# ctpeterson/qex

Hardware: AMD Instinct MI355X
Metric: staggered Dslash GFLOP/s + CG iters/s, 32^4 SU(3) fp64, 1/2/4/8 MI355X (higher is better)
Workload: dtype f64

## Files before the change

qex_amd/csrc/dslash.hip:

```cpp
#include "qexhip_internal.h"
#include "site_index.h"
#include "reduce.h"
#include "fused_sweep.h"
#include <hip/hip_ext.h>
#include <cstring>
#include <algorithm>
#include <chrono>

static double now_us() { return std::chrono::duration<double, std::micro>(std::chrono::steady_clock::now().time_since_epoch()).count(); }

struct DslashArgs {
  Geom g;
  const double2 *W;
  const unsigned long long *S;
  const double2 *in;
  double2 *out;
  const double2 *rin;
  const double2 *xs;
  double ca, cb;
  double sgn;
  double post;
  int parity, c0, c1;
  int d0, d1, nb1;
  const double2 *gh_hi, *gh_lo;
  double *partials;
  const int *done;
  int swz;
  int ntstore;
  FusedSweep fs;
};

#include "dslash_core.h"

template <int NDIR, bool HALO, bool INIT, bool DOT, int RECON, bool FUSED>
__device__ __forceinline__ void dslash_body(const DslashArgs &A) {
  const bool skip = A.done && *A.done;
  if (skip && !FUSED) return;
  if (FUSED && fused_push(A.fs, skip)) return;
  FusedRole R;
  R.bid = blockIdx.x; R.cleanup = false; R.bnd = false; R.parked = false;
  if (FUSED) fused_enter(A.fs, A.nb1, R);
  const bool cleanup = FUSED && R.cleanup;
  for (;;) {
    int lb = R.bid;
    if (FUSED && !fused_next_block(A.fs, R, lb)) break;
    const bool bnd = FUSED && R.bnd;
    if (A.swz && !bnd) {
      int per = A.swz >> 3;
      lb = (lb & 7) * per + (lb >> 3);
    }
    int c = A.c0 + lb * 256 + threadIdx.x;
    int clim = A.c1;
    if (FUSED) c = fused_site(A.fs, R, lb, A.c0, A.c1, A.d0, A.d1, clim);
    else if (lb >= A.nb1) { c = A.d0 + (lb - A.nb1) * 256 + threadIdx.x; clim = A.d1; }
    double dotv = 0;
    const bool active = c < clim && !skip;
    const Geom &g = A.g;
    const SiteXYZT s = site_coord(g, c, A.parity);
    const int tu = FUSED ? __builtin_amdgcn_readfirstlane(s.t) : 0;
    double2 acc[3];
    double2 xsv[3];
    constexpr int NLOAD = (RECON == 1 || RECON == 3) ? 6 : (RECON == 2 ? 7 : 9);
    constexpr int LROW = RECON == 3 ? LR_ROW : NLOAD * 64;
    const double2 *w = A.W + (size_t)(c >> 6) * (NDIR * LROW) + (c & 63);
    const unsigned long long *sm = RECON == 1 ? A.S + (size_t)(c >> 6) * NDIR : (RECON == 3 ? A.S + (size_t)(c >> 6) * NDIR * 2 : nullptr);
    const double2 *in_f1 = A.in, *in_b1 = A.in, *in_f3 = A.in, *in_b3 = A.in;
    if (FUSED) {
      in_f1 = tu + 1 >= g.X[3] ? A.gh_hi : A.in;
      in_b1 = tu - 1 < 0 ? A.gh_lo : A.in;
      in_f3 = tu + 3 >= g.X[3] ? A.gh_hi : A.in;
      in_b3 = tu - 3 < 0 ? A.gh_lo : A.in;
    }
    auto pair = [&](const int pr, const bool do_f, const bool do_b) __attribute__((always_inline)) {
      const int mu = pr & 3;
      const int hop = pr >= 4 ? 3 : 1;
      const int pf = nbr_pos<HALO>(g, c, s, mu, hop);
      const int pb = nbr_pos<HALO>(g, c, s, mu, -hop);
      const double2 *wp = w + (size_t)pr * (2 * LROW);
      double2 U[9], W[9], vf[3], vb[3];
      if (do_f) {
#pragma unroll
        for (int k = 0; k < NLOAD; k++) {
          d2v t = __builtin_nontemporal_load((const d2v *)&wp[k * 64]);
          U[k] = make_double2(t.x, t.y);
        }
      }
      if (do_b) {
#pragma unroll
        for (int k = 0; k < NLOAD; k++) {
          d2v t = __builtin_nontemporal_load((const d2v *)&wp[LROW + k * 64]);
          W[k] = make_double2(t.x, t.y);
        }
      }
      if (RECON == 1) {
        const int lane = c & 63;
        if (do_f) recon_row2<1>(U, (sm[2 * pr] >> lane) & 1ull);
        if (do_b) recon_row2<1>(W, (sm[2 * pr + 1] >> lane) & 1ull);
      } else if (RECON == 3) {
        const int lane = c & 63;
        const size_t fr = ((size_t)(c >> 6) * NDIR + 2 * pr) * 576 + lane;
        if (do_f) recon_row2_res(U, wp - lane, sm + 4 * pr, A.S - 2, fr, lane);
        if (do_b) recon_row2_res(W, wp - lane + LROW, sm + 4 * pr + 2, A.S - 2, fr + 576, lane);
      } else if (RECON == 2) {
        if (do_f) recon_row2<2>(U, false);
        if (do_b) recon_row2<2>(W, false);
      }
      const double2 *srcf = (FUSED && mu == 3) ? (hop == 3 ? in_f3 : in_f1) : A.in;
      const double2 *srcb = (FUSED && mu == 3) ? (hop == 3 ? in_b3 : in_b1) : A.in;
      if (do_f) {
#pragma unroll
        for (int k = 0; k < 3; k++) vf[k] = srcf[vec_off(pf, k)];
      }
      if (do_b) {
#pragma unroll
        for (int k = 0; k < 3; k++) vb[k] = srcb[vec_off(pb, k)];
      }
      if (do_f) mv3<false>(acc, U, vf);
      if (do_b) mv3<true>(acc, W, vb);
    };
    auto edge_pairs = [&](const bool crossing) __attribute__((always_inline)) {
      if (!crossing) {
        constexpr int NSP = NDIR / 2 - NDIR / 8;
        constexpr int UNS = NDIR == 8 ? 1 : 2;
#pragma unroll UNS
        for (int q = 0; q < NSP; q++) pair(q + q / 3, true, true);
      }
#pragma unroll 1
      for (int pr = 3; pr < NDIR / 2; pr += 4) {
        const int hop = pr >= 4 ? 3 : 1;
        const bool xf = tu + hop >= g.X[3], xb = tu - hop < 0;
        pair(pr, crossing ? xf : !xf, crossing ? xb : !xb);
      }
    };
    const bool edge = FUSED && bnd;
    if (active) {
      if ((INIT && !cleanup) || DOT) {
#pragma unroll
        for (int k = 0; k < 3; k++) xsv[k] = A.xs[vec_off(c, k)];
      }
      if (FUSED && cleanup) {
#pragma unroll
        for (int k = 0; k < 3; k++) acc[k] = A.out[vec_off(c, k)];
      } else if (INIT) {
#pragma unroll
        for (int k = 0; k < 3; k++) {
          acc[k].x = (A.sgn * A.cb) * xsv[k].x;
          acc[k].y = (A.sgn * A.cb) * xsv[k].y;
        }
        if (A.ca != 0.0) {
#pragma unroll
          for (int k = 0; k < 3; k++) {
            double2 r = A.rin[vec_off(c, k)];
            acc[k].x += (A.sgn * A.ca) * r.x;
            acc[k].y += (A.sgn * A.ca) * r.y;
          }
        }
      } else {
#pragma unroll
        for (int k = 0; k < 3; k++) acc[k] = make_double2(0.0, 0.0);
      }
      constexpr int UNR = (NDIR == 8) ? (RECON == 3 ? (FUSED ? 1 : 2) : (RECON ? 1 : 4)) : 2;
      if (!edge) {
#pragma unroll UNR
        for (int pr = 0; pr < NDIR / 2; pr++) pair(pr, true, true);
      } else if (!cleanup) {
        edge_pairs(false);
      }
    }
    if (edge && !skip) {
      fused_wait_faces(A.fs, R);
      if (active && !R.parked) edge_pairs(true);
    }
    const bool parked = FUSED && R.parked;
    if (active) {
      if (parked) {
#pragma unroll
        for (int k = 0; k < 3; k++) A.out[vec_off(c, k)] = acc[k];
      } else {
#pragma unroll
        for (int k = 0; k < 3; k++) {
          acc[k].x *= (A.sgn * A.post); acc[k].y *= (A.sgn * A.post);
          if (A.ntstore) {
            d2v t; t.x = acc[k].x; t.y = acc[k].y;
            __builtin_nontemporal_store(t, (d2v *)&A.out[vec_off(c, k)]);
          } else {
            A.out[vec_off(c, k)] = acc[k];
          }
        }
        if (DOT) {
#pragma unroll
          for (int k = 0; k < 3; k++) dotv = fma(xsv[k].x, acc[k].x, fma(xsv[k].y, acc[k].y, dotv));
        }
      }
    }
    if (DOT && !skip && !parked) {
      const int pidx = !FUSED ? (RECON == 3 ? lb : (int)blockIdx.x) : fused_partial_slot(A.fs, R, lb);
      double r = block_sum_256(dotv);
      if (threadIdx.x == 0) A.partials[pidx] = r;
    }
    if (!cleanup) break;
  }
  if (FUSED) fused_finish(A.fs, R);
}

template <int NDIR, bool HALO, bool INIT, bool DOT, int RECON>
__global__ void __launch_bounds__(256) k_dslash(DslashArgs A) { dslash_body<NDIR, HALO, INIT, DOT, RECON, false>(A); }
template <int NDIR, bool INIT, bool DOT, int RECON>
__global__ void __launch_bounds__(256) k_dslash_fused(DslashArgs A) { dslash_body<NDIR, true, INIT, DOT, RECON, true>(A); }

template <class K>
static void launch_timed(qexhip_ctx *c, const char *tname, K kernel, dim3 grid, dim3 block, DslashArgs &A, hipStream_t st) {
  hipEvent_t e0 = nullptr, e1 = nullptr;
  if (timer_event_pair(c, tname, &e0, &e1)) hipExtLaunchKernelGGL(kernel, grid, block, 0, st, e0, e1, 0, A);
  else hipLaunchKernelGGL(kernel, grid, block, 0, st, A);
}

template <int NDIR, bool HALO>
static int launch(qexhip_ctx *c, DslashArgs &A, int c0, int c1, bool init, bool dot, int part_off,
                  int d0 = 0, int d1 = 0, const char *tname = "dslash", hipStream_t st = nullptr, int fused_grid = 0) {
  if (!st) st = c->stream;
  const bool fused = fused_grid > 0;
  if (c1 <= c0 && d1 <= d0) return 0;
  if (c1 <= c0) { c0 = d0; c1 = d1; d0 = d1 = 0; }
  A.c0 = c0; A.c1 = c1; A.d0 = d0; A.d1 = d1;
  A.nb1 = (c1 - c0 + 255) / 256;
  const int nb = A.nb1 + (d1 > d0 ? (d1 - d0 + 255) / 256 : 0);
  const int nsw = fused ? A.nb1 : nb;
  A.swz = ((c->recon != 0 || (c->lres && !fused)) && nsw >= 64 && (nsw & 7) == 0) ? nsw : 0;
  A.ntstore = 1;
  double *psave = A.partials;
  A.partials = psave ? psave + part_off : nullptr;
  dim3 grid(fused ? fused_grid : nb), block(256);
#define QX_LAUNCH(R) \
  do { \
    if (HALO && fused) { \
      if (init && dot) launch_timed(c, tname, k_dslash_fused<NDIR, true, true, R>, grid, block, A, st); \
      else if (init) launch_timed(c, tname, k_dslash_fused<NDIR, true, false, R>, grid, block, A, st); \
      else if (dot) launch_timed(c, tname, k_dslash_fused<NDIR, false, true, R>, grid, block, A, st); \
      else launch_timed(c, tname, k_dslash_fused<NDIR, false, false, R>, grid, block, A, st); \
    } else if (init && dot) launch_timed(c, tname, k_dslash<NDIR, HALO, true, true, R>, grid, block, A, st); \
    else if (init) launch_timed(c, tname, k_dslash<NDIR, HALO, true, false, R>, grid, block, A, st); \
    else if (dot) launch_timed(c, tname, k_dslash<NDIR, HALO, false, true, R>, grid, block, A, st); \
    else launch_timed(c, tname, k_dslash<NDIR, HALO, false, false, R>, grid, block, A, st); \
  } while (0)
  if (c->recon == 1) QX_LAUNCH(1);
  else if (c->recon == 2) QX_LAUNCH(2);
  else if constexpr (NDIR == 8) {
    if (c->lres) QX_LAUNCH(3);
    else QX_LAUNCH(0);
  } else QX_LAUNCH(0);
#undef QX_LAUNCH
  A.partials = psave;
  HIPCHK(hipGetLastError());
  return 0;
}

void sweep_plan(const qexhip_ctx *c, int *lo_end_out, int *hi_beg_out, int *overlap_out) {
  const Geom &g = c->g;
  int lo_end = g.depth * g.F; if (lo_end > g.Vh) lo_end = g.Vh;
  int hi_beg = g.Vh - g.depth * g.F; if (hi_beg < lo_end) hi_beg = lo_end;
  const size_t face_bytes = (size_t)g.depth * g.F * 48;
  *lo_end_out = lo_end; *hi_beg_out = hi_beg;
  const int tuned = c->overlap_auto[c->ndir == 16];
  *overlap_out = !g.halo || hi_beg <= lo_end ? 0
                 : (c->opt_overlap >= 0 ? (c->opt_overlap != 0)
                    : (tuned >= 0 ? tuned : ((hi_beg - lo_end) >= 131072 && face_bytes >= ((size_t)1 << 20))));
}

int sweep_form(const qexhip_ctx *c, int overlap) {
  if (!overlap || !peer_faces(c)) return 0;
  if (c->opt_hop_split >= 0) return c->opt_hop_split ? 2 : 0;
  const int m = c->form_auto[c->ndir == 16];
  return m >= 0 ? m : 2;
}

static double exchange_estimate_us(const qexhip_ctx *c) {
  const double meas = c->xchg_us[c->ndir == 16];
  if (meas > 0) return meas;
  const double link = (c->emu_link_gbs > 0 ? c->emu_link_gbs : 45.0) * 1e3;
  return 3.0 + (double)c->g.depth * c->g.F * 48.0 / link;
}
double sweep_push_fraction(const qexhip_ctx *c, int interior_sites, int nrhs) {
  const double bsite = c->ndir * (c->recon == 1 ? 96.0 : (c->recon == 2 ? 112.0 : (c->lres ? 108.0 : 144.0))) + 120.0 * nrhs;
  const double t_int = (double)interior_sites * bsite / 5.5e6;
  return t_int > 0 ? std::min(1.0, std::max(0.65, nrhs * exchange_estimate_us(c) / t_int)) : 1.0;
}

static int sweep_fused_ctl(qexhip_ctx *c, int nbnd, FusedCtl *F, int nrhs) {
  if (c->fz_cap < nbnd) {
    HIPCHK(hipStreamSynchronize(c->stream));
    if (c->fz_buf) HIPCHK(hipFree(c->fz_buf));
    c->fz_buf = nullptr; c->fz_cap = 0;
    const int cap = std::max(2 * nbnd, 4096);
    HIPCHK(hipMalloc((void **)&c->fz_buf, (size_t)(256 + cap) * sizeof(unsigned int)));
    HIPCHK(hipMemsetAsync(c->fz_buf, 0, (size_t)(256 + cap) * sizeof(unsigned int), c->stream));
    c->fz_cap = cap;
  }
  F->dec = c->fz_buf; F->ndef = c->fz_buf + 32; F->cl_done = c->fz_buf + 64; F->late = c->fz_buf + 96;
  F->list = c->fz_buf + 256;
  F->ncl = std::max(std::min(nbnd, 4), std::min(nbnd / 8, 32));
  const double tick_per_us = (double)c->dj.ticks / (c->dj.timeout_s * 1e6);
  if (c->opt_fused_spin_us == -2) F->spin_ticks = -1;
  else {
    const double us = c->opt_fused_spin_us >= 0 ? (double)c->opt_fused_spin_us : std::max(25.0, nrhs * exchange_estimate_us(c));
    F->spin_ticks = (long long)(us * tick_per_us);
  }
  return 0;
}

int fused_sweep_setup(qexhip_ctx *c, int nrhs, DevField *const *f, int parity, int lo_end, int hi_beg, FusedSweep *F,
                      const double2 **gh_hi, const double2 **gh_lo, int *grid, int *nparts) {
  const int nb_int = (hi_beg - lo_end + 255) / 256, nb_lo = (lo_end + 255) / 256, nb_hi = (c->g.Vh - hi_beg + 255) / 256;
  CHK(comm_halo_push_only_multi(c, nrhs, f, parity, gh_hi, gh_lo, &F->push));
  CHK(peer_ghost_args(c, &F->pg));
  CHK(sweep_fused_ctl(c, nb_lo + nb_hi, &F->fz, nrhs));
  F->e0 = hi_beg; F->e1 = c->g.Vh; F->nb2 = nb_int + nb_lo;
  F->nbA = (int)(sweep_push_fraction(c, hi_beg - lo_end, nrhs) * nb_int);
// ... 162 lines not shown
```

qex_amd/csrc/dslash_core.h:

```cpp
#pragma once
#include <hip/hip_runtime.h>
#include "link_residual.h"

typedef double d2v __attribute__((ext_vector_type(2)));

template <bool SUB>
__device__ __forceinline__ void mv3(double2 acc[3], const double2 U[9], const double2 v[3]) {
#pragma unroll
  for (int i = 0; i < 3; i++) {
#pragma unroll
    for (int j = 0; j < 3; j++) {
      if (!SUB) {
        acc[i].x += U[3 * i + j].x * v[j].x;
        acc[i].x -= U[3 * i + j].y * v[j].y;
        acc[i].y += U[3 * i + j].x * v[j].y;
        acc[i].y += U[3 * i + j].y * v[j].x;
      } else {
        acc[i].x -= U[3 * i + j].x * v[j].x;
        acc[i].x += U[3 * i + j].y * v[j].y;
        acc[i].y -= U[3 * i + j].x * v[j].y;
        acc[i].y -= U[3 * i + j].y * v[j].x;
      }
    }
  }
}

template <int FMT>
__device__ __forceinline__ void recon_row2(double2 U[9], bool neg) {
  const double2 ph = U[6];
  double2 r2[3];
#pragma unroll
  for (int k = 0; k < 3; k++) {
    const int a = (k + 1) % 3, b = (k + 2) % 3;
    double rx = U[a].x * U[3 + b].x;
    rx -= U[a].y * U[3 + b].y;
    rx -= U[b].x * U[3 + a].x;
    rx += U[b].y * U[3 + a].y;
    double ry = U[b].x * U[3 + a].y;
    ry += U[b].y * U[3 + a].x;
    ry -= U[a].x * U[3 + b].y;
    ry -= U[a].y * U[3 + b].x;
    if (FMT == 1) r2[k] = make_double2(neg ? -rx : rx, neg ? -ry : ry);
    else r2[k] = make_double2(fma(ph.x, rx, -(ph.y * ry)), fma(ph.x, ry, ph.y * rx));
  }
#pragma unroll
  for (int k = 0; k < 3; k++) U[6 + k] = r2[k];
}

__device__ __forceinline__ void recon_row2_res(double2 U[9], const double2 *row, const unsigned long long *m, const unsigned long long *hdr,
                                               size_t fr, int lane) {
  const uint64_t lo = __builtin_nontemporal_load((const uint64_t *)(row + LR_RES) + lane);
  const uint32_t hi = __builtin_nontemporal_load((const uint32_t *)(row + LR_RES + 32) + lane);
  double2 r2[3];
  lr_decode(U, (m[0] >> lane) & 1ull, lo, hi, r2);
  if ((m[1] >> lane) & 1ull) {
    const double2 *wf = (const double2 *)(uintptr_t)hdr[0] + fr;
#pragma unroll
    for (int k = 0; k < 3; k++) r2[k] = wf[(6 + k) * 64];
  }
#pragma unroll
  for (int k = 0; k < 3; k++) U[6 + k] = r2[k];
}

template <int RECON>
__device__ __forceinline__ void load_link(double2 U[9], const double2 *w, const unsigned long long *sm, int lane) {
  constexpr int NLOAD = RECON == 1 ? 6 : (RECON == 2 ? 7 : 9);
#pragma unroll
  for (int k = 0; k < NLOAD; k++) U[k] = w[k * 64];
  if (RECON == 1) recon_row2<1>(U, (*sm >> lane) & 1ull);
  else if (RECON == 2) recon_row2<2>(U, false);
}
```

qex_amd/csrc/layout.hip:

```cpp
#include <algorithm>
#include <vector>
#include "qexhip_internal.h"
#include "site_index.h"
#include "link_residual.h"
#include <cstring>

int geom_init(Geom &g, const int X[4], int depth, int halo) {
  for (int i = 0; i < 4; i++) {
    if (X[i] < 2 || (X[i] & 1)) { qexhip_set_error("local lattice extents must be even and >= 2 (got %d in dim %d)", X[i], i); return -1; }
    if (X[i] > 1024) { qexhip_set_error("local lattice extents above 1024 are not supported (got %d in dim %d)", X[i], i); return -1; }
    g.X[i] = X[i];
  }
  g.Xh = X[0] / 2;
  g.V = X[0] * X[1] * X[2] * X[3];
  g.Vh = g.V / 2;
  g.F = g.Xh * X[1] * X[2];
  g.ntile = (g.Vh + QEXHIP_TILE - 1) / QEXHIP_TILE;
  g.halo = halo;
  g.depth = halo ? depth : 0;
  if (halo) {
    if (g.F % QEXHIP_TILE) { qexhip_set_error("sharding in t needs X*Y*Z/2 to be a multiple of 64 (got %d)", g.F); return -1; }
    if (X[3] < 3) { qexhip_set_error("sharding in t needs a local t extent >= 3"); return -1; }
    g.gtile = 3 * g.F / QEXHIP_TILE;
  } else {
// ... 37 lines not shown

int field_upload(qexhip_ctx *c, DevField &f, const double *host) {
  size_t bytes = (size_t)c->g.V * 6 * sizeof(double);
  CHK(ensure_stage(c, bytes));
  HIPCHK(hipMemcpyAsync(c->stage, host, bytes, hipMemcpyHostToDevice, c->stream));
  k_vec_to_tiles<<<(c->g.V + 255) / 256, 256, 0, c->stream>>>(c->g, (const double2 *)c->stage, f.d, f.half);
  HIPCHK(hipGetLastError());
  return 0;
}

int field_download(qexhip_ctx *c, const DevField &f, double *host) {
  size_t bytes = (size_t)c->g.V * 6 * sizeof(double);
  CHK(ensure_stage(c, bytes));
  k_vec_from_tiles<<<(c->g.V + 255) / 256, 256, 0, c->stream>>>(c->g, (double2 *)c->stage, f.d, f.half);
  HIPCHK(hipGetLastError());
  HIPCHK(hipMemcpyAsync(host, c->stage, bytes, hipMemcpyDeviceToHost, c->stream));
  HIPCHK(hipStreamSynchronize(c->stream));
  return 0;
}

__global__ void __launch_bounds__(256) k_pack_top_links(Geom g, const double2 *__restrict__ hostfmt, double2 *buf) {
  int n = g.depth * g.F;
  int i = blockIdx.x * 256 + threadIdx.x;
  if (i >= 2 * n) return;
  int p = i / n, j = i - p * n;
  int c = g.Vh - n + j;
  const double2 *U = hostfmt + ((size_t)(p * g.Vh + c) * 4 + 3) * 9;
  for (int k = 0; k < 9; k++) buf[(size_t)i * 9 + k] = U[k];
}

template <bool HALO>
__global__ void __launch_bounds__(256) k_links_to_tiles(Geom g, const double2 *__restrict__ hostfmt,
                                                        const double2 *__restrict__ ghost, double2 *W,
                                                        int ndir, int dbase, int hop) {
  int i = blockIdx.x * 256 + threadIdx.x;
  if (i >= g.V) return;
  int p = i >= g.Vh, c = i - p * g.Vh;
  SiteXYZT s = site_coord(g, c, p);
  double2 *w = W + ((size_t)p * g.ntile + (c >> 6)) * ndir * 576 + (c & 63);
  for (int mu = 0; mu < 4; mu++) {
    const double2 *U = hostfmt + ((size_t)i * 4 + mu) * 9;
    double2 *wf = w + (size_t)(dbase + 2 * mu) * 576;
    for (int k = 0; k < 9; k++) wf[k * 64] = U[k];
    const double2 *B;
    if (HALO && mu == 3 && s.t - hop < 0) {
      int cF = c - s.t * g.F;
      int j = (s.t - hop + g.depth) * g.F + cF;
      B = ghost + ((size_t)(1 - p) * g.depth * g.F + j) * 9;
    } else {
      int cb = nbr_pos<false>(g, c, s, mu, -hop);
      B = hostfmt + ((size_t)((1 - p) * g.Vh + cb) * 4 + mu) * 9;
    }
    double2 *wb = w + (size_t)(dbase + 2 * mu + 1) * 576;
    for (int r = 0; r < 3; r++)
      for (int q = 0; q < 3; q++) {
        double2 v = B[q * 3 + r];
        wb[(r * 3 + q) * 64] = make_double2(v.x, -v.y);
      }
  }
}

int links_upload(qexhip_ctx *c, const double *fat, const double *lng) {
  c->cg_resume.valid = 0;
  const Geom &g = c->g;
  int ndir = lng ? 16 : 8;
  if (lng) for (int i = 0; i < 4; i++) if (g.X[i] < 4) { qexhip_set_error("Naik links need local extents >= 4"); return -1; }
  if (lng && g.halo && g.depth < 3) { qexhip_set_error("internal: ghost depth %d < 3 for Naik links", g.depth); return -3; }
  size_t wbytes = (size_t)2 * g.ntile * ndir * 576 * sizeof(double2);
  if (c->W && c->ndir != ndir) { HIPCHK(hipFree(c->W)); c->W = nullptr; }
  if (!c->W) { HIPCHK(hipMalloc((void **)&c->W, wbytes)); }
  HIPCHK(hipMemsetAsync(c->W, 0, wbytes, c->stream));
  c->ndir = ndir;
  size_t gbytes = (size_t)g.V * 72 * sizeof(double);
  size_t ghost_elems = g.halo ? (size_t)2 * g.depth * g.F * 9 : 0;
  size_t ghost_bytes = ghost_elems * sizeof(double2);
  CHK(ensure_stage(c, gbytes + 2 * ghost_bytes + 256));
  double2 *hostfmt = (double2 *)c->stage;
  double2 *sendbuf = (double2 *)((char *)c->stage + gbytes);
  double2 *ghost = (double2 *)((char *)c->stage + gbytes + ghost_bytes);
  for (int pass = 0; pass < (lng ? 2 : 1); pass++) {
    const double *src = pass ? lng : fat;
    HIPCHK(hipMemcpyAsync(hostfmt, src, gbytes, hipMemcpyHostToDevice, c->stream));
    if (g.halo) {
      int n = 2 * g.depth * g.F;
      k_pack_top_links<<<(n + 255) / 256, 256, 0, c->stream>>>(g, hostfmt, sendbuf);
      HIPCHK(hipGetLastError());
      CHK(comm_exchange_raw(c, sendbuf, ghost, ghost_bytes, c->stream));
      k_links_to_tiles<true><<<(g.V + 255) / 256, 256, 0, c->stream>>>(g, hostfmt, ghost, c->W, ndir, pass * 8, pass ? 3 : 1);
    } else {
      k_links_to_tiles<false><<<(g.V + 255) / 256, 256, 0, c->stream>>>(g, hostfmt, nullptr, c->W, ndir, pass * 8, pass ? 3 : 1);
    }
    HIPCHK(hipGetLastError());
  }
  HIPCHK(hipStreamSynchronize(c->stream));
  CHK(links_compress(c));
  return sweep_autotune(c);
}

template <int FMT>
__global__ void __launch_bounds__(256) k_links_compress(size_t nrows, const double2 *__restrict__ W, double2 *Wc,
                                                        unsigned long long *Ws, unsigned int *maxdev) {
  const size_t j = (size_t)blockIdx.x * 256 + threadIdx.x;
  const size_t row = j >> 6;
  if (row >= nrows) return;
  const int l = j & 63;
  const double2 *w = W + row * 576 + l;
  constexpr int NR = FMT == 1 ? 6 : 7;
  double2 *o = Wc + row * (NR * 64) + l;
  double2 u[9], r[3];
#pragma unroll
  for (int k = 0; k < 9; k++) u[k] = w[k * 64];
#pragma unroll
  for (int k = 0; k < 6; k++) o[k * 64] = u[k];
  double n2 = 0, px = 0, py = 0;
#pragma unroll
  for (int k = 0; k < 3; k++) {
    const int a = (k + 1) % 3, b = (k + 2) % 3;
    r[k].x = (u[a].x * u[3 + b].x - u[a].y * u[3 + b].y) - (u[b].x * u[3 + a].x - u[b].y * u[3 + a].y);
    r[k].y = -((u[a].x * u[3 + b].y + u[a].y * u[3 + b].x) - (u[b].x * u[3 + a].y + u[b].y * u[3 + a].x));
    n2 += r[k].x * r[k].x + r[k].y * r[k].y;
    px += u[6 + k].x * r[k].x + u[6 + k].y * r[k].y;
    py += u[6 + k].y * r[k].x - u[6 + k].x * r[k].y;
  }
  double2 ph;
  if (n2 > 0) ph = make_double2(px / n2, py / n2); else ph = make_double2(1.0, 0.0);
  if (FMT == 1) ph = make_double2(ph.x < 0 ? -1.0 : 1.0, 0.0);
  double dev = 0;
#pragma unroll
  for (int k = 0; k < 3; k++) {
    const double rx = ph.x * r[k].x - ph.y * r[k].y, ry = ph.x * r[k].y + ph.y * r[k].x;
    dev = fmax(dev, fmax(fabs(u[6 + k].x - rx), fabs(u[6 + k].y - ry)));
  }
  if (FMT == 1) {
    const unsigned long long mask = __ballot(ph.x < 0);
    if (l == 0) Ws[row] = mask;
  } else {
    o[6 * 64] = ph;
  }
  unsigned int bits = __float_as_uint((float)dev);
#pragma unroll
  for (int off = 32; off > 0; off >>= 1) {
    const unsigned int o2 = __shfl_xor(bits, off, 64);
    bits = o2 > bits ? o2 : bits;
  }
  if (l == 0 && bits > __hip_atomic_load(maxdev, __ATOMIC_RELAXED, __HIP_MEMORY_SCOPE_AGENT)) atomicMax(maxdev, bits);
}
__global__ void __launch_bounds__(256) k_links_residual(size_t nrows, size_t prows, const double2 *__restrict__ W, double2 *Wc,
                                                        unsigned long long *Wm, unsigned int *nesc) {
  const size_t j = (size_t)blockIdx.x * 256 + threadIdx.x;
  const size_t row = j >> 6;
  if (row >= nrows) return;
  const int l = j & 63;
  const double2 *w = W + row * 576 + l;
  double2 *o = Wc + row * LR_ROW + l;
  double2 u[9];
#pragma unroll
  for (int k = 0; k < 9; k++) u[k] = w[k * 64];
#pragma unroll
  for (int k = 0; k < 6; k++) o[k * 64] = u[k];
  bool neg;
  uint64_t lo;
  uint32_t hi;
  const bool ok = lr_encode(u, &neg, &lo, &hi);
  ((uint64_t *)(Wc + row * LR_ROW + LR_RES))[l] = lo;
  ((uint32_t *)(Wc + row * LR_ROW + LR_RES + 32))[l] = hi;
  const unsigned long long sgn = __ballot(neg), esc = __ballot(!ok);
  if (l == 0) {
    unsigned long long *m = Wm + 2 * (row + row / prows + 1);
    m[0] = sgn;
    m[1] = esc;
    if (esc) atomicAdd(nesc, (unsigned int)__popcll(esc));
  }
}

int link_residual_host(const double2 *u, long n, unsigned char *escaped, double2 *row2) {
  for (long i = 0; i < n; i++) {
    bool neg;
    uint64_t lo;
    uint32_t hi;
    const bool ok = lr_encode(u + 9 * i, &neg, &lo, &hi);
    if (escaped) escaped[i] = !ok;
    if (row2) lr_decode(u + 9 * i, neg, lo, hi, row2 + 3 * i);
  }
  return 0;
}

int links_compress(qexhip_ctx *c) {
  const Geom &g = c->g;
  c->links_gen++;
  c->recon = 0;
  c->lres = 0; c->lres_esc = 0;
  if (!c->opt_recon || !c->W) return 0;
  const size_t nrows = (size_t)2 * g.ntile * c->ndir;
  if (c->Wc_rows < nrows) {
    if (c->Wc) HIPCHK(hipFree(c->Wc));
    if (c->Ws) HIPCHK(hipFree(c->Ws));
    HIPCHK(hipMalloc((void **)&c->Wc, nrows * 448 * sizeof(double2)));
    HIPCHK(hipMalloc((void **)&c->Ws, nrows * sizeof(unsigned long long)));
    c->Wc_rows = nrows;
  }
  unsigned int *flag = (unsigned int *)&c->dscal[62];
  const unsigned nblk = (unsigned)((nrows * 64 + 255) / 256);
  for (int fmt = 1; fmt <= 2; fmt++) {
    if (fmt == 2 && c->opt_recon == 1) break;
    HIPCHK(hipMemsetAsync(flag, 0, sizeof(unsigned int), c->stream));
    if (fmt == 1) k_links_compress<1><<<nblk, 256, 0, c->stream>>>(nrows, c->W, c->Wc, c->Ws, flag);
    else k_links_compress<2><<<nblk, 256, 0, c->stream>>>(nrows, c->W, c->Wc, c->Ws, flag);
    HIPCHK(hipGetLastError());
    unsigned int bits = 0;
    HIPCHK(hipMemcpyAsync(&bits, flag, sizeof(bits), hipMemcpyDeviceToHost, c->stream));
    HIPCHK(hipStreamSynchronize(c->stream));
    float dev;
    memcpy(&dev, &bits, sizeof(dev));
    if (fmt == 1 || dev <= 5e-14f) c->recon_dev = dev;
    if (dev <= 5e-14f) { c->recon = fmt; break; }
  }
  if (!c->recon && c->opt_lossless && c->ndir == 8) {
    if (!c->Wm || c->Wm_rows < nrows) {
      if (c->Wm) HIPCHK(hipFree(c->Wm));
      c->Wm = nullptr; c->Wm_rows = 0;
      HIPCHK(hipMalloc((void **)&c->Wm, (nrows + 2) * 2 * sizeof(unsigned long long)));
      c->Wm_rows = nrows;
    }
    const size_t prows = nrows / 2;
    HIPCHK(hipMemsetAsync(flag, 0, sizeof(unsigned int), c->stream));
    k_links_residual<<<nblk, 256, 0, c->stream>>>(nrows, prows, c->W, c->Wc, c->Wm, flag);
    HIPCHK(hipGetLastError());
    unsigned int nesc = 0;
    HIPCHK(hipMemcpyAsync(&nesc, flag, sizeof(nesc), hipMemcpyDeviceToHost, c->stream));
    const unsigned long long hdr[2][2] = {{(unsigned long long)(uintptr_t)c->W, 0}, {(unsigned long long)(uintptr_t)(c->W + prows * 576), 0}};
    for (int p = 0; p < 2; p++) HIPCHK(hipMemcpyAsync(c->Wm + p * 2 * (prows + 1), hdr[p], sizeof hdr[p], hipMemcpyHostToDevice, c->stream));
    HIPCHK(hipStreamSynchronize(c->stream));
    c->lres_esc = nesc;
    if ((double)nesc <= 0.01 * (double)(nrows * 64)) c->lres = 1;
  }
  return 0;
}

__global__ void __launch_bounds__(256) k_links_from_nat(Geom g, const double2 *__restrict__ N, double2 *W, int ndir, int dbase, int hop) {
  int i = blockIdx.x * 256 + threadIdx.x;
  if (i >= g.V) return;
  int p = i >= g.Vh, c = i - p * g.Vh;
  SiteXYZT s = site_coord(g, c, p);
  double2 *w = W + ((size_t)p * g.ntile + (c >> 6)) * ndir * 576 + (c & 63);
  for (int mu = 0; mu < 4; mu++) {
    const double2 *U = N + (((size_t)p * g.etile + (c >> 6)) * 4 + mu) * 576 + (c & 63);
    double2 *wf = w + (size_t)(dbase + 2 * mu) * 576;
    for (int k = 0; k < 9; k++) wf[k * 64] = U[k * 64];
    int cb;
    if (g.halo && mu == 3) {
      const int t = c / g.F, tn = t - hop;
      cb = (tn < 0 ? tn + g.X[3] + 6 : tn) * g.F + (c - t * g.F);
    } else {
      cb = nbr_pos<false>(g, c, s, mu, -hop);
    }
    const double2 *B = N + (((size_t)(1 - p) * g.etile + (cb >> 6)) * 4 + mu) * 576 + (cb & 63);
    double2 *wb = w + (size_t)(dbase + 2 * mu + 1) * 576;
    for (int r = 0; r < 3; r++)
      for (int q = 0; q < 3; q++) {
        double2 v = B[(q * 3 + r) * 64];
        wb[(r * 3 + q) * 64] = make_double2(v.x, -v.y);
      }
  }
}
int links_from_natural(qexhip_ctx *c, const double2 *fat, const double2 *lng) {
  c->cg_resume.valid = 0;
  const Geom &g = c->g;
  int ndir = lng ? 16 : 8;
  if (lng) for (int i = 0; i < 4; i++) if (g.X[i] < 4) { qexhip_set_error("Naik links need local extents >= 4"); return -1; }
  if (g.halo) c->g.depth = lng ? 3 : 1;
  size_t wbytes = (size_t)2 * g.ntile * ndir * 576 * sizeof(double2);
  if (c->W && c->ndir != ndir) { HIPCHK(hipFree(c->W)); c->W = nullptr; }
  if (!c->W) { HIPCHK(hipMalloc((void **)&c->W, wbytes)); }
  HIPCHK(hipMemsetAsync(c->W, 0, wbytes, c->stream));
  c->ndir = ndir;
  k_links_from_nat<<<(g.V + 255) / 256, 256, 0, c->stream>>>(g, fat, c->W, ndir, 0, 1);
  if (lng) k_links_from_nat<<<(g.V + 255) / 256, 256, 0, c->stream>>>(g, lng, c->W, ndir, 8, 3);
  HIPCHK(hipGetLastError());
  HIPCHK(hipStreamSynchronize(c->stream));
  CHK(links_compress(c));
  return sweep_autotune(c);
}

extern "C" int qexhip_debug_geom(const int latLocal[4], int depth, int halo, int out[8]) {
  Geom g;
  if (geom_init(g, latLocal, depth, halo)) return -1;
  out[0] = g.Vh; out[1] = g.F; out[2] = g.ntile; out[3] = g.gtile; out[4] = g.etile;
  out[5] = g.depth; out[6] = g.halo; out[7] = g.Xh;
  return 0;
}
extern "C" int qexhip_debug_nbr_pos(const int latLocal[4], int depth, int halo, int c, int parity, int mu, int hop) {
  Geom g;
  if (geom_init(g, latLocal, depth, halo)) return -1;
  if (c < 0 || c >= g.Vh || mu < 0 || mu > 3) return -1;
  SiteXYZT s = site_coord(g, c, parity);
  return halo ? nbr_pos<true>(g, c, s, mu, hop) : nbr_pos<false>(g, c, s, mu, hop);
}
extern "C" int qexhip_debug_site_coord(const int latLocal[4], int c, int parity, int x[4]) {
  Geom g;
  if (geom_init(g, latLocal, 1, 0)) return -1;
  if (c < 0 || c >= g.Vh) return -1;
  SiteXYZT s = site_coord(g, c, parity);
  x[0] = 2 * s.xh + s.o; x[1] = s.y; x[2] = s.z; x[3] = s.t;
  return 0;
}

int tile_order_table(qexhip_ctx *c, const int **tab, int *chunk_out) {
  const Geom &g = c->g;
  const int n = 2 * g.ntile, chunk = (n + 7) / 8;
  if (c->tile_order && c->tile_order_n == 8 * chunk) { *tab = c->tile_order; *chunk_out = chunk; return 0; }
  constexpr int by = 8, bz = 4, bt = 4;
  struct Ent { unsigned long long key0, key1; int e; };
  std::vector<Ent> v(n);
  for (int p = 0; p < 2; p++)
    for (int tile = 0; tile < g.ntile; tile++) {
      unsigned r = (unsigned)tile * 64u / (unsigned)g.Xh;
      const int y = r % g.X[1]; r /= g.X[1];
      const int z = r % g.X[2], t = r / g.X[2];
// ... 98 lines not shown
```

qex_amd/csrc/link_residual.h:

```cpp
#pragma once
#include <hip/hip_runtime.h>
#include <cstdint>
#include <cmath>

#define LR_ROW 432
#define LR_RES 384

__host__ __device__ __forceinline__ uint64_t lr_bits(double x) { return __builtin_bit_cast(uint64_t, x); }
__host__ __device__ __forceinline__ double lr_double(uint64_t b) { return __builtin_bit_cast(double, b); }

__host__ __device__ __forceinline__ void lr_rebuild(const double2 u[6], bool neg, double rec[6]) {
#pragma clang fp contract(off)
#pragma unroll
  for (int k = 0; k < 3; k++) {
    const int a = (k + 1) % 3, b = (k + 2) % 3;
    double rx = u[a].x * u[3 + b].x;
    rx = fma(-u[a].y, u[3 + b].y, rx);
    rx = fma(-u[b].x, u[3 + a].x, rx);
    rx = fma(u[b].y, u[3 + a].y, rx);
    double ry = u[b].x * u[3 + a].y;
    ry = fma(u[b].y, u[3 + a].x, ry);
    ry = fma(-u[a].x, u[3 + b].y, ry);
    ry = fma(-u[a].y, u[3 + b].x, ry);
    rec[2 * k] = neg ? -rx : rx;
    rec[2 * k + 1] = neg ? -ry : ry;
  }
}

__host__ __device__ __forceinline__ double lr_apply(double rec, int k) {
  const double sc = lr_double(lr_bits(rec) & 0x7ff0000000000000ull) * 0x1p-52;
  return fma((double)k, sc, rec);
}

__host__ __device__ __forceinline__ void lr_decode(const double2 u[6], bool neg, uint64_t lo, uint32_t hi, double2 r2[3]) {
  double rec[6];
  lr_rebuild(u, neg, rec);
  const int k[6] = {(int16_t)lo, (int16_t)(lo >> 16), (int16_t)(lo >> 32), (int16_t)(lo >> 48), (int16_t)hi, (int16_t)(hi >> 16)};
#pragma unroll
  for (int j = 0; j < 3; j++) r2[j] = make_double2(lr_apply(rec[2 * j], k[2 * j]), lr_apply(rec[2 * j + 1], k[2 * j + 1]));
}

__host__ __device__ __forceinline__ bool lr_encode(const double2 u[9], bool *neg, uint64_t *lo, uint32_t *hi) {
  double rec[6];
  lr_rebuild(u, false, rec);
  double px = 0;
#pragma unroll
  for (int j = 0; j < 3; j++) px += u[6 + j].x * rec[2 * j] + u[6 + j].y * rec[2 * j + 1];
  const bool ng = px < 0;
  if (ng) {
#pragma unroll
    for (int j = 0; j < 6; j++) rec[j] = -rec[j];
  }
  const double row2[6] = {u[6].x, u[6].y, u[7].x, u[7].y, u[8].x, u[8].y};
  int k[6];
  bool ok = true;
#pragma unroll
  for (int j = 0; j < 6; j++) {
    const double sc = lr_double(lr_bits(rec[j]) & 0x7ff0000000000000ull) * 0x1p-52;
    const double q = sc > 0 ? (row2[j] - rec[j]) / sc : 0.0;
    k[j] = fabs(q) <= 32767.0 ? (int)rint(q) : 0;
    ok = ok && lr_bits(lr_apply(rec[j], k[j])) == lr_bits(row2[j]);
  }
  if (!ok) {
#pragma unroll
    for (int j = 0; j < 6; j++) k[j] = 0;
  }
  *neg = ng;
  *lo = (uint64_t)(uint16_t)k[0] | (uint64_t)(uint16_t)k[1] << 16 | (uint64_t)(uint16_t)k[2] << 32 | (uint64_t)(uint16_t)k[3] << 48;
  *hi = (uint32_t)(uint16_t)k[4] | (uint32_t)(uint16_t)k[5] << 16;
  return ok;
}
```

Before: 2866.

## Interleave forward/backward link residuals and hoist escape-row loads out of the decode path

Link storage for RECON==3 changes from separate forward and backward rows to a paired block. The forward and backward 2x6 rows sit first, and their residual words are interleaved so one vector nontemporal load fetches both. The per-tile sign and escape masks are read once through the constant address space into registers. Escaped third-row loads are done ahead of time, and a branch-free bitmask select replaces the divergent escape branch. The aim is fewer load instructions, scalarized mask traffic and less divergence, at the cost of more registers and unconditional escape selects.

```diff
diff --git a/qex_amd/csrc/dslash.hip b/qex_amd/csrc/dslash.hip
--- a/qex_amd/csrc/dslash.hip
+++ b/qex_amd/csrc/dslash.hip
@@ -62,8 +62,11 @@
     double2 xsv[3];
     constexpr int NLOAD = (RECON == 1 || RECON == 3) ? 6 : (RECON == 2 ? 7 : 9);
     constexpr int LROW = RECON == 3 ? LR_ROW : NLOAD * 64;
-    const double2 *w = A.W + (size_t)(c >> 6) * (NDIR * LROW) + (c & 63);
-    const unsigned long long *sm = RECON == 1 ? A.S + (size_t)(c >> 6) * NDIR : (RECON == 3 ? A.S + (size_t)(c >> 6) * NDIR * 2 : nullptr);
+    const int tile = RECON == 3 ? __builtin_amdgcn_readfirstlane(c >> 6) : (c >> 6);
+    const double2 *w = A.W + (size_t)tile * (NDIR * LROW) + (c & 63);
+    const unsigned long long *sm = RECON == 1 ? A.S + (size_t)(c >> 6) * NDIR : nullptr;
+    LrTile lt;
+    LrEsc le0;
     const double2 *in_f1 = A.in, *in_b1 = A.in, *in_f3 = A.in, *in_b3 = A.in;
     if (FUSED) {
       in_f1 = tu + 1 >= g.X[3] ? A.gh_hi : A.in;
@@ -71,7 +74,7 @@
       in_f3 = tu + 3 >= g.X[3] ? A.gh_hi : A.in;
       in_b3 = tu - 3 < 0 ? A.gh_lo : A.in;
     }
-    auto pair = [&](const int pr, const bool do_f, const bool do_b) __attribute__((always_inline)) {
+    auto pair = [&](const int pr, const bool do_f, const bool do_b, const LrEsc &le) __attribute__((always_inline)) {
       const int mu = pr & 3;
       const int hop = pr >= 4 ? 3 : 1;
       const int pf = nbr_pos<HALO>(g, c, s, mu, hop);
@@ -88,7 +91,7 @@
       if (do_b) {
 #pragma unroll
         for (int k = 0; k < NLOAD; k++) {
-          d2v t = __builtin_nontemporal_load((const d2v *)&wp[LROW + k * 64]);
+          d2v t = __builtin_nontemporal_load((const d2v *)&wp[(RECON == 3 ? LR_BWD : LROW) + k * 64]);
           W[k] = make_double2(t.x, t.y);
         }
       }
@@ -98,9 +101,10 @@
         if (do_b) recon_row2<1>(W, (sm[2 * pr + 1] >> lane) & 1ull);
       } else if (RECON == 3) {
         const int lane = c & 63;
-        const size_t fr = ((size_t)(c >> 6) * NDIR + 2 * pr) * 576 + lane;
-        if (do_f) recon_row2_res(U, wp - lane, sm + 4 * pr, A.S - 2, fr, lane);
-        if (do_b) recon_row2_res(W, wp - lane + LROW, sm + 4 * pr + 2, A.S - 2, fr + 576, lane);
+        const lr_u64x2 lo = __builtin_nontemporal_load((const lr_u64x2 *)&wp[LR_RES]);
+        const lr_u32x2 hi = __builtin_nontemporal_load((const lr_u32x2 *)(wp - lane + LR_RES + 64) + lane);
+        if (do_f) lr_row2(U, lr_mask(lt, pr, 0), lr_mask(lt, pr, 1), lo.x, hi.x, le.f, lane);
+        if (do_b) lr_row2(W, lr_mask(lt, pr, 2), lr_mask(lt, pr, 3), lo.y, hi.y, le.b, lane);
       } else if (RECON == 2) {
         if (do_f) recon_row2<2>(U, false);
         if (do_b) recon_row2<2>(W, false);
@@ -123,17 +127,22 @@
         constexpr int NSP = NDIR / 2 - NDIR / 8;
         constexpr int UNS = NDIR == 8 ? 1 : 2;
 #pragma unroll UNS
-        for (int q = 0; q < NSP; q++) pair(q + q / 3, true, true);
+        for (int q = 0; q < NSP; q++) {
+          if constexpr (RECON == 3) lr_escaped_rows<NDIR>(le0, lt, tile, q + q / 3, c & 63, true, true);
+          pair(q + q / 3, true, true, le0);
+        }
       }
 #pragma unroll 1
       for (int pr = 3; pr < NDIR / 2; pr += 4) {
         const int hop = pr >= 4 ? 3 : 1;
         const bool xf = tu + hop >= g.X[3], xb = tu - hop < 0;
-        pair(pr, crossing ? xf : !xf, crossing ? xb : !xb);
+        if constexpr (RECON == 3) lr_escaped_rows<NDIR>(le0, lt, tile, pr, c & 63, crossing ? xf : !xf, crossing ? xb : !xb);
+        pair(pr, crossing ? xf : !xf, crossing ? xb : !xb, le0);
       }
     };
     const bool edge = FUSED && bnd;
     if (active) {
+      if (RECON == 3) lr_tile_masks(lt, A.S, tile);
       if ((INIT && !cleanup) || DOT) {
 #pragma unroll
         for (int k = 0; k < 3; k++) xsv[k] = A.xs[vec_off(c, k)];
@@ -160,9 +169,18 @@
         for (int k = 0; k < 3; k++) acc[k] = make_double2(0.0, 0.0);
       }
       constexpr int UNR = (NDIR == 8) ? (RECON == 3 ? (FUSED ? 1 : 2) : (RECON ? 1 : 4)) : 2;
-      if (!edge) {
+      if (!edge && RECON == 3) {
+#pragma unroll 1
+        for (int p0 = 0; p0 < NDIR / 2; p0 += UNR) {
+          LrEsc le[UNR];
+#pragma unroll
+          for (int q = 0; q < UNR; q++) lr_escaped_rows<NDIR>(le[q], lt, tile, p0 + q, c & 63, true, true);
+#pragma unroll
+          for (int q = 0; q < UNR; q++) pair(p0 + q, true, true, le[q]);
+        }
+      } else if (!edge) {
 #pragma unroll UNR
-        for (int pr = 0; pr < NDIR / 2; pr++) pair(pr, true, true);
+        for (int pr = 0; pr < NDIR / 2; pr++) pair(pr, true, true, le0);
       } else if (!cleanup) {
         edge_pairs(false);
       }
diff --git a/qex_amd/csrc/dslash_core.h b/qex_amd/csrc/dslash_core.h
--- a/qex_amd/csrc/dslash_core.h
+++ b/qex_amd/csrc/dslash_core.h
@@ -47,19 +47,55 @@
   for (int k = 0; k < 3; k++) U[6 + k] = r2[k];
 }
 
-__device__ __forceinline__ void recon_row2_res(double2 U[9], const double2 *row, const unsigned long long *m, const unsigned long long *hdr,
-                                               size_t fr, int lane) {
-  const uint64_t lo = __builtin_nontemporal_load((const uint64_t *)(row + LR_RES) + lane);
-  const uint32_t hi = __builtin_nontemporal_load((const uint32_t *)(row + LR_RES + 32) + lane);
+typedef const __attribute__((address_space(4))) unsigned long long *lr_cmask_p;
+typedef unsigned long long lr_u64x2 __attribute__((ext_vector_type(2)));
+typedef unsigned int lr_u32x2 __attribute__((ext_vector_type(2)));
+
+struct LrTile {
+  unsigned long long m[16];
+  const double2 *w18;
+};
+__device__ __forceinline__ void lr_tile_masks(LrTile &T, const unsigned long long *S, int tile) {
+  const lr_cmask_p p = (lr_cmask_p)(S + (size_t)tile * 16);
+#pragma unroll
+  for (int j = 0; j < 16; j++) T.m[j] = p[j];
+  T.w18 = (const double2 *)(uintptr_t)((lr_cmask_p)(S - 2))[0];
+}
+__device__ __forceinline__ unsigned long long lr_mask(const LrTile &T, int pr, int j) {
+  const unsigned long long a = pr & 1 ? T.m[4 + j] : T.m[j], b = pr & 1 ? T.m[12 + j] : T.m[8 + j];
+  const unsigned long long r = pr & 2 ? b : a;
+  return r;
+}
+
+struct LrEsc { double2 f[3], b[3]; };
+template <int NDIR>
+__device__ __forceinline__ void lr_escaped_rows(LrEsc &E, const LrTile &T, int tile, int pr, int lane, bool do_f, bool do_b) {
+  typedef const __attribute__((address_space(1))) d2v *gp;
+  const gp wf = (gp)T.w18 + ((size_t)tile * NDIR + 2 * pr) * 576 + lane;
+#pragma unroll
+  for (int k = 0; k < 3; k++) E.f[k] = E.b[k] = make_double2(0.0, 0.0);
+  const unsigned long long ef = lr_mask(T, pr, 1), eb = lr_mask(T, pr, 3);
+  if (do_f && ef != 0) {
+    const gp q = wf - (((ef >> lane) & 1ull) ? 0 : lane);
+#pragma unroll
+    for (int k = 0; k < 3; k++) { const d2v t = q[(6 + k) * 64]; E.f[k] = make_double2(t.x, t.y); }
+  }
+  if (do_b && eb != 0) {
+    const gp q = wf + 576 - (((eb >> lane) & 1ull) ? 0 : lane);
+#pragma unroll
+    for (int k = 0; k < 3; k++) { const d2v t = q[(6 + k) * 64]; E.b[k] = make_double2(t.x, t.y); }
+  }
+}
+
+__device__ __forceinline__ void lr_row2(double2 U[9], unsigned long long sign, unsigned long long esc, uint64_t lo, uint32_t hi,
+                                        const double2 e[3], int lane) {
   double2 r2[3];
-  lr_decode(U, (m[0] >> lane) & 1ull, lo, hi, r2);
-  if ((m[1] >> lane) & 1ull) {
-    const double2 *wf = (const double2 *)(uintptr_t)hdr[0] + fr;
+  lr_decode(U, (sign >> lane) & 1ull, lo, hi, r2);
+  unsigned long long x = 0ull - ((esc >> lane) & 1ull);
+  asm("" : "+v"(x));
 #pragma unroll
-    for (int k = 0; k < 3; k++) r2[k] = wf[(6 + k) * 64];
-  }
-#pragma unroll
-  for (int k = 0; k < 3; k++) U[6 + k] = r2[k];
+  for (int k = 0; k < 3; k++)
+    U[6 + k] = make_double2(lr_double((lr_bits(e[k].x) & x) | (lr_bits(r2[k].x) & ~x)), lr_double((lr_bits(e[k].y) & x) | (lr_bits(r2[k].y) & ~x)));
 }
 
 template <int RECON>
diff --git a/qex_amd/csrc/layout.hip b/qex_amd/csrc/layout.hip
--- a/qex_amd/csrc/layout.hip
+++ b/qex_amd/csrc/layout.hip
@@ -213,7 +213,9 @@
   if (row >= nrows) return;
   const int l = j & 63;
   const double2 *w = W + row * 576 + l;
-  double2 *o = Wc + row * LR_ROW + l;
+  const int fb = row & 1;
+  double2 *pb = Wc + (row >> 1) * LR_PAIR;
+  double2 *o = pb + fb * LR_BWD + l;
   double2 u[9];
 #pragma unroll
   for (int k = 0; k < 9; k++) u[k] = w[k * 64];
@@ -223,8 +225,8 @@
   uint64_t lo;
   uint32_t hi;
   const bool ok = lr_encode(u, &neg, &lo, &hi);
-  ((uint64_t *)(Wc + row * LR_ROW + LR_RES))[l] = lo;
-  ((uint32_t *)(Wc + row * LR_ROW + LR_RES + 32))[l] = hi;
+  ((uint64_t *)(pb + LR_RES))[2 * l + fb] = lo;
+  ((uint32_t *)(pb + LR_RES + 64))[2 * l + fb] = hi;
   const unsigned long long sgn = __ballot(neg), esc = __ballot(!ok);
   if (l == 0) {
     unsigned long long *m = Wm + 2 * (row + row / prows + 1);
diff --git a/qex_amd/csrc/link_residual.h b/qex_amd/csrc/link_residual.h
--- a/qex_amd/csrc/link_residual.h
+++ b/qex_amd/csrc/link_residual.h
@@ -4,7 +4,9 @@
 #include <cmath>
 
 #define LR_ROW 432
-#define LR_RES 384
+#define LR_PAIR 864
+#define LR_BWD 384
+#define LR_RES 768
 
 __host__ __device__ __forceinline__ uint64_t lr_bits(double x) { return __builtin_bit_cast(uint64_t, x); }
 __host__ __device__ __forceinline__ double lr_double(uint64_t b) { return __builtin_bit_cast(double, b); }
```

Measured after the change: 2871, median of 3. About the same (+0.2%).

## Prefetch residual-link escape rows and masks ahead of decode in two-slot pipeline

Applied to the files above, without the earlier changes.

For the residual-compressed link format in the non-fused path, the escape-row loads and per-wave sign/escape masks are issued in a first phase for two direction pairs before any link decode happens. The escape-row latency then overlaps the main link and vector loads instead of sitting behind a divergent branch inside the decode. The escape patch is applied with a branchless bitwise select, and the mask base pointer is made wave-uniform via readfirstlane so the masks can go through scalar loads. This holds extra registers for the prefetched escape values, and the edge/cleanup branching is bypassed for this format, which could raise register pressure or lower occupancy.

```diff
diff --git a/qex_amd/csrc/dslash.hip b/qex_amd/csrc/dslash.hip
--- a/qex_amd/csrc/dslash.hip
+++ b/qex_amd/csrc/dslash.hip
@@ -63,7 +63,8 @@
     constexpr int NLOAD = (RECON == 1 || RECON == 3) ? 6 : (RECON == 2 ? 7 : 9);
     constexpr int LROW = RECON == 3 ? LR_ROW : NLOAD * 64;
     const double2 *w = A.W + (size_t)(c >> 6) * (NDIR * LROW) + (c & 63);
-    const unsigned long long *sm = RECON == 1 ? A.S + (size_t)(c >> 6) * NDIR : (RECON == 3 ? A.S + (size_t)(c >> 6) * NDIR * 2 : nullptr);
+    const unsigned long long *sm = RECON == 1 ? A.S + (size_t)(c >> 6) * NDIR
+                                   : (RECON == 3 ? A.S + (size_t)__builtin_amdgcn_readfirstlane(c >> 6) * (NDIR * 2) : nullptr);
     const double2 *in_f1 = A.in, *in_b1 = A.in, *in_f3 = A.in, *in_b3 = A.in;
     if (FUSED) {
       in_f1 = tu + 1 >= g.X[3] ? A.gh_hi : A.in;
@@ -71,13 +72,27 @@
       in_f3 = tu + 3 >= g.X[3] ? A.gh_hi : A.in;
       in_b3 = tu - 3 < 0 ? A.gh_lo : A.in;
     }
-    auto pair = [&](const int pr, const bool do_f, const bool do_b) __attribute__((always_inline)) {
+    unsigned long long em[2][4];
+    double2 ee[2][2][3];
+    auto pair = [&](const int pr, const bool do_f, const bool do_b, const int phase = 0, const int slot = 0) __attribute__((always_inline)) {
       const int mu = pr & 3;
       const int hop = pr >= 4 ? 3 : 1;
       const int pf = nbr_pos<HALO>(g, c, s, mu, hop);
       const int pb = nbr_pos<HALO>(g, c, s, mu, -hop);
       const double2 *wp = w + (size_t)pr * (2 * LROW);
       double2 U[9], W[9], vf[3], vb[3];
+      unsigned long long *m = em[slot];
+      double2 *ef = ee[slot][0], *eb = ee[slot][1];
+      if (RECON == 3 && phase != 2) {
+        const int lane = c & 63;
+        typedef const double2 __attribute__((address_space(1))) *gptr;
+        const double2 *wf = (const double2 *)(gptr)(uintptr_t)A.S[-2] + ((size_t)(c >> 6) * NDIR + 2 * pr) * 576 + lane;
+#pragma unroll
+        for (int k = 0; k < 4; k++) m[k] = sm[4 * pr + k];
+        if (do_f) lr_escape_load(ef, m[1], wf, lane);
+        if (do_b) lr_escape_load(eb, m[3], wf + 576, lane);
+      }
+      if (phase == 1) return;
       if (do_f) {
 #pragma unroll
         for (int k = 0; k < NLOAD; k++) {
@@ -98,9 +113,8 @@
         if (do_b) recon_row2<1>(W, (sm[2 * pr + 1] >> lane) & 1ull);
       } else if (RECON == 3) {
         const int lane = c & 63;
-        const size_t fr = ((size_t)(c >> 6) * NDIR + 2 * pr) * 576 + lane;
-        if (do_f) recon_row2_res(U, wp - lane, sm + 4 * pr, A.S - 2, fr, lane);
-        if (do_b) recon_row2_res(W, wp - lane + LROW, sm + 4 * pr + 2, A.S - 2, fr + 576, lane);
+        if (do_f) recon_row2_res(U, wp - lane, m[0], m[1], ef, lane);
+        if (do_b) recon_row2_res(W, wp - lane + LROW, m[2], m[3], eb, lane);
       } else if (RECON == 2) {
         if (do_f) recon_row2<2>(U, false);
         if (do_b) recon_row2<2>(W, false);
@@ -160,7 +174,15 @@
         for (int k = 0; k < 3; k++) acc[k] = make_double2(0.0, 0.0);
       }
       constexpr int UNR = (NDIR == 8) ? (RECON == 3 ? (FUSED ? 1 : 2) : (RECON ? 1 : 4)) : 2;
-      if (!edge) {
+      if (RECON == 3 && !FUSED) {
+#pragma unroll 1
+        for (int pr = 0; pr < NDIR / 2; pr += 2) {
+          pair(pr, true, true, 1, 0);
+          pair(pr + 1, true, true, 1, 1);
+          pair(pr, true, true, 2, 0);
+          pair(pr + 1, true, true, 2, 1);
+        }
+      } else if (!edge) {
 #pragma unroll UNR
         for (int pr = 0; pr < NDIR / 2; pr++) pair(pr, true, true);
       } else if (!cleanup) {
diff --git a/qex_amd/csrc/dslash_core.h b/qex_amd/csrc/dslash_core.h
--- a/qex_amd/csrc/dslash_core.h
+++ b/qex_amd/csrc/dslash_core.h
@@ -47,19 +47,29 @@
   for (int k = 0; k < 3; k++) U[6 + k] = r2[k];
 }
 
-__device__ __forceinline__ void recon_row2_res(double2 U[9], const double2 *row, const unsigned long long *m, const unsigned long long *hdr,
-                                               size_t fr, int lane) {
+__device__ __forceinline__ void lr_escape_load(double2 e[3], unsigned long long esc, const double2 *wf, int lane) {
+#pragma unroll
+  for (int k = 0; k < 3; k++) e[k] = make_double2(0.0, 0.0);
+  if (esc != 0) {
+    if ((esc >> lane) & 1ull) {
+#pragma unroll
+      for (int k = 0; k < 3; k++) e[k] = wf[(6 + k) * 64];
+    }
+  }
+}
+
+__device__ __forceinline__ void recon_row2_res(double2 U[9], const double2 *row, unsigned long long sign, unsigned long long esc,
+                                               const double2 e[3], int lane) {
   const uint64_t lo = __builtin_nontemporal_load((const uint64_t *)(row + LR_RES) + lane);
   const uint32_t hi = __builtin_nontemporal_load((const uint32_t *)(row + LR_RES + 32) + lane);
   double2 r2[3];
-  lr_decode(U, (m[0] >> lane) & 1ull, lo, hi, r2);
-  if ((m[1] >> lane) & 1ull) {
-    const double2 *wf = (const double2 *)(uintptr_t)hdr[0] + fr;
+  lr_decode(U, (sign >> lane) & 1ull, lo, hi, r2);
+  unsigned int mk = 0u - ((unsigned int)(esc >> lane) & 1u);
+  asm("" : "+v"(mk));
+  const uint64_t mk2 = (uint64_t)mk << 32 | mk;
 #pragma unroll
-    for (int k = 0; k < 3; k++) r2[k] = wf[(6 + k) * 64];
-  }
-#pragma unroll
-  for (int k = 0; k < 3; k++) U[6 + k] = r2[k];
+  for (int k = 0; k < 3; k++)
+    U[6 + k] = make_double2(lr_double((lr_bits(e[k].x) & mk2) | (lr_bits(r2[k].x) & ~mk2)), lr_double((lr_bits(e[k].y) & mk2) | (lr_bits(r2[k].y) & ~mk2)));
 }
 
 template <int RECON>
```

Result: slower. 2849 before, 2748 after (-3.6%).
